# tjysdsg/speech-recognition

Hardware: AMD Instinct MI355X
Metric: frame-state loglik/s + utterances/s Viterbi decode (higher is better)
Workload: dtype f64; 1 GPU; configs[1]: 10-digit HMM, 5 states/digit, 8-mix GMM, 39-dim, 10000 utterances/GPU (999364 frames on rank 0), isolated-word decode; states=50, mixtures=8, dim=39, parallelism=utterance-sharded x1, batches_in_flight=2, process_group=single

## Files before the change

include/gmmhmm.h:

```cpp
#ifndef GMMHMM_H
#define GMMHMM_H

#include <stdint.h>

#ifdef __cplusplus
extern "C" {
#endif

typedef enum {
    GH_OK = 0,
    GH_ERR_INVALID = -1,
    GH_ERR_HIP = -2,
    GH_ERR_NOMEM = -3,
    GH_ERR_NODEVICE = -4,
    GH_ERR_SELF_POINTER = -5,
    GH_ERR_UNSUPPORTED = -6,
    GH_ERR_COMM = -7
} gh_status;

typedef enum { GH_F32 = 0, GH_F64 = 1 } gh_dtype;

typedef struct gh_ctx gh_ctx;
typedef struct gh_gmm gh_gmm;
typedef struct gh_batch gh_batch;
// ... 71 lines not shown
void* gh_loglik_dev_ptr(gh_batch* b);
int gh_loglik_fetch(gh_ctx* ctx, const gh_batch* b, void* out_host );
int gh_component_loglik(gh_ctx* ctx, const gh_gmm* g, int state, int64_t N,
                        const double* x_host , double* out_host );
int gh_distance_matrix(gh_ctx* ctx, int64_t N, int K, int D, const double* x_host ,
                       const double* y_host , const double* var_host, int var_rows,
                       double* out_host );

int gh_lattices_create(gh_ctx* ctx, int L,
                       const int64_t* row_off , const int32_t* row_state,
                       const int64_t* arc_off , const int32_t* arc_to,
                       const int32_t* arc_from, const double* arc_cost,
                       const int64_t* start_off , const int32_t* start_rows,
                       const int64_t* end_off , const int32_t* end_rows,
                       gh_lattices** out);
int gh_lattices_create_transcripts(gh_ctx* ctx, int W, int n, const double* word_trans ,
                                   const int32_t* state_base , int64_t L,
                                   const int64_t* label_off , const int32_t* labels, gh_lattices** out);
void gh_lattices_destroy(gh_lattices* l);
int gh_lattices_set_beam(gh_lattices* l, int beam);

int gh_lattices_forms(const gh_lattices* l);

int gh_viterbi(gh_ctx* ctx, const gh_lattices* lat, const gh_batch* b,
               const int32_t* utt_lattice ,
               double* out_end_cost, int32_t* out_best_end,
               int32_t* out_path, const int64_t* path_off , int32_t* out_path_len,
               double* out_costs, const int64_t* costs_off );
int gh_viterbi_fused(gh_ctx* ctx, const gh_gmm* g, const gh_lattices* lat, gh_batch* b, int log_domain,
                     double* out_end_cost, int32_t* out_best_end,
                     int32_t* out_path, const int64_t* path_off , int32_t* out_path_len,
                     double* out_costs, const int64_t* costs_off );
int gh_ctx_last_fused(const gh_ctx* ctx);
int64_t gh_viterbi_path_cap(const gh_lattices* lat, int l, int64_t T);
int gh_viterbi_labels(gh_ctx* ctx, const gh_lattices* lat, const gh_batch* b,
                      const int32_t* utt_lattice , const int32_t* row_label,
                      double* out_end_cost, int32_t* out_best_end,
                      int32_t* out_labels, const int64_t* label_off , int32_t* out_n_labels);
int gh_viterbi_labels_timed(gh_ctx* ctx, const gh_lattices* lat, const gh_batch* b,
                            const int32_t* utt_lattice , const int32_t* row_label,
                            double* out_end_cost, int32_t* out_best_end,
                            int32_t* out_labels, const int64_t* label_off , int32_t* out_n_labels,
                            int32_t* out_begin );

#define GH_SEGMENT_START (1 << 30)
int gh_align_segments(gh_ctx* ctx, const gh_lattices* lat, const gh_batch* b,
                      const int32_t* utt_lattice ,
                      double* out_end_cost, int32_t* out_best_end, int32_t* out_frame_state );
int gh_align_runs(gh_ctx* ctx, const gh_lattices* lat, const gh_batch* b, const int32_t* utt_lattice ,
                  double* out_end_cost, int32_t* out_best_end, int run_cap, int32_t* out_runs ,
                  int32_t* out_run_cnt );

int gh_viterbi_labels_packed(gh_ctx* ctx, const gh_lattices* lat, const gh_batch* b,
                             const int32_t* utt_lattice , const int32_t* row_label, int max_labels,
                             double* out_end_cost, int32_t* out_best_end,
                             int32_t* out_labels, int64_t out_capacity, int32_t* out_n_labels);
int gh_viterbi_labels_packed_timed(gh_ctx* ctx, const gh_lattices* lat, const gh_batch* b,
                                   const int32_t* utt_lattice , const int32_t* row_label, int max_labels,
                                   double* out_end_cost, int32_t* out_best_end,
                                   int32_t* out_labels, int64_t out_capacity, int32_t* out_n_labels,
                                   int32_t* out_begin );

int gh_dtw(gh_ctx* ctx, const gh_batch* b, int n, const double* y, const double* var,
           const double* trans, int beam, const double* dist_host,
           double* out_costs, int32_t* out_path, int32_t* out_path_len);

// ... 165 lines not shown
```

speech-recognition_amd/csrc/gh_decode.hip:

```cpp
#include "gh_internal.h"
#include <chrono>
#include <string>
#include "gh_host.h"
#include "gh_viterbi.h"
#include "gh_dtw.h"
#include "gh_fb.h"

namespace {

template <bool TIMED>
__device__ __forceinline__ void path_labels_walk(const int32_t* __restrict__ path, const int64_t* __restrict__ path_off,
                                                 const int32_t* __restrict__ path_len, const int32_t* __restrict__ utt_lat,
                                                 const gh_lattices::desc* __restrict__ descs,
                                                 const int32_t* __restrict__ row_label,
                                                 const int64_t* __restrict__ label_off, int32_t* __restrict__ labels,
                                                 int32_t* __restrict__ n_labels, int* __restrict__ flag,
                                                 int32_t* __restrict__ begins) {
    const int64_t u = blockIdx.x;
    const int lane = threadIdx.x;
    const int len = path_len[u];
    const int32_t* p = path + 2 * path_off[u];
    const int32_t* lab = row_label + descs[utt_lat ? utt_lat[u] : 0].row_base;
    const int64_t cap = label_off[u + 1] - label_off[u];
    int32_t* out = labels + label_off[u];
// ... 548 lines not shown
    }
    return GH_OK;
}

extern "C" int gh_viterbi(gh_ctx* ctx, const gh_lattices* lat, const gh_batch* b, const int32_t* utt_lattice,
                          double* out_end_cost, int32_t* out_best_end, int32_t* out_path,
                          const int64_t* path_off, int32_t* out_path_len, double* out_costs,
                          const int64_t* costs_off) {
    return viterbi_impl(ctx, lat, b, utt_lattice, out_end_cost, out_best_end, out_path, path_off, out_path_len, out_costs,
                        costs_off, nullptr, nullptr, nullptr, nullptr);
}

extern "C" int gh_viterbi_fused(gh_ctx* ctx, const gh_gmm* g, const gh_lattices* lat, gh_batch* b, int log_domain,
                                double* out_end_cost, int32_t* out_best_end, int32_t* out_path, const int64_t* path_off,
                                int32_t* out_path_len, double* out_costs, const int64_t* costs_off) {
    GH_REQUIRE(ctx && g && lat && b, "gh_viterbi_fused: NULL argument");
    GH_REQUIRE(g->D == b->D || b->N == 0, "gh_viterbi_fused: model has %d dimensions, batch %d", g->D, b->D);
    ctx->last_fused = 0;
    bool can = g->M == 1 && lat->chain_ok && lat->beam <= 0 && forced_kernel() == 0 && gh_fused_dv(g->D) > 0 && !lat->deferred_src;
    if (const char* e = getenv("GMMHMM_FUSED")) can = can && atoi(e) != 0;
    if (b->any_T1) can = false;
    if (!can) {
        const int compat = ctx->compat;
        if (log_domain) ctx->compat &= ~1;
        const int rc = gh_loglik(ctx, g, b, nullptr);
        ctx->compat = compat;
        if (rc) return rc;
    }
    return viterbi_impl(ctx, lat, b, nullptr, out_end_cost, out_best_end, out_path, path_off, out_path_len, out_costs, costs_off,
                        nullptr, nullptr, nullptr, nullptr, -1, nullptr, can ? g : nullptr, log_domain);
}

extern "C" int gh_ctx_last_fused(const gh_ctx* ctx) { return ctx ? ctx->last_fused : -1; }

extern "C" int gh_viterbi_labels_timed(gh_ctx* ctx, const gh_lattices* lat, const gh_batch* b, const int32_t* utt_lattice,
                                       const int32_t* row_label, double* out_end_cost, int32_t* out_best_end,
                                       int32_t* out_labels, const int64_t* label_off, int32_t* out_n_labels, int32_t* out_begin) {
    GH_REQUIRE(row_label && out_labels && label_off && out_n_labels, "gh_viterbi_labels: NULL argument");
    return viterbi_impl(ctx, lat, b, utt_lattice, out_end_cost, out_best_end, nullptr, nullptr, nullptr, nullptr, nullptr,
                        row_label, out_labels, label_off, out_n_labels, -1, nullptr, nullptr, 0, 0, nullptr, nullptr, out_begin);
}

extern "C" int gh_viterbi_labels(gh_ctx* ctx, const gh_lattices* lat, const gh_batch* b, const int32_t* utt_lattice,
                                 const int32_t* row_label, double* out_end_cost, int32_t* out_best_end,
                                 int32_t* out_labels, const int64_t* label_off, int32_t* out_n_labels) {
    return gh_viterbi_labels_timed(ctx, lat, b, utt_lattice, row_label, out_end_cost, out_best_end, out_labels, label_off, out_n_labels,
                                   nullptr);
}

extern "C" int gh_dtw(gh_ctx* ctx, const gh_batch* b, int n, const double* y, const double* var,
                      const double* trans, int beam, const double* dist_host, double* out_costs,
                      int32_t* out_path, int32_t* out_path_len) {
    GH_REQUIRE(ctx && b && trans, "gh_dtw: NULL argument");
    GH_REQUIRE(dist_host || y, "gh_dtw: need template rows or a distance matrix");
    GH_REQUIRE(n > 1 && n <= 1024, "gh_dtw: n=%d (2..1024 supported; decode.py:22 asserts n > 1)", n);
    GH_REQUIRE(b->dtype == GH_F64 || dist_host, "gh_dtw: built-in distances need an fp64 batch");
    GH_REQUIRE(!out_path || out_path_len, "gh_dtw: out_path needs out_path_len");
    GH_HIP(hipSetDevice(ctx->device));
    const int64_t U = b->U, N = b->N;
    const int D = b->D;
    if (U == 0) return GH_OK;
    for (int64_t u = 0; u < U; ++u)
        GH_REQUIRE(b->offsets[u + 1] - b->offsets[u] > 1, "gh_dtw: utterance %lld has fewer than 2 frames (decode.py:22)",
                   (long long)u);
    std::vector<double> logdet(n, 0.0);
    if (var && !dist_host)
// ... 344 lines not shown
```

speech-recognition_amd/csrc/gh_internal.h:

```cpp
#pragma once
#include <hip/hip_runtime.h>
#include <stdint.h>
#include <stdarg.h>
#include <stdio.h>
#include <string>
#include <vector>
#include "../../include/gmmhmm.h"

void gh_set_error(const char* fmt, ...);

#define GH_HIP(call)                                                                     \
    do {                                                                                 \
        hipError_t e_ = (call);                                                          \
        if (e_ != hipSuccess) {                                                          \
            gh_set_error("%s:%d %s -> %s", __FILE__, __LINE__, #call, hipGetErrorString(e_)); \
            return (e_ == hipErrorOutOfMemory) ? GH_ERR_NOMEM : GH_ERR_HIP;              \
        }                                                                                \
    } while (0)

#define GH_REQUIRE(cond, ...)                 \
    do {                                      \
        if (!(cond)) {                        \
            gh_set_error(__VA_ARGS__);        \
            return GH_ERR_INVALID;            \
        }                                     \
    } while (0)

#define GH_LEAN_NARROW_ARCS 3

#define GH_LSE_SCALE64 184.66496523378731614
#define GH_LSE_SCALE32 1.4426950408889634074
#define GH_LSE_OFF64 (-1e300)
#define GH_LSE_OFF32 (-1e30f)

struct gh_ctx {
    int device;
    hipStream_t stream;
    int n_cu;
    void* scratch;
    size_t scratch_bytes;
    int* d_flag;
    void* pinned;
    size_t pinned_bytes;
    double* d_fp64_tables;
    int compat;
    int last_fused = 0;
    int last_chunks;
    size_t budget_cache = 0;
    int budget_age = 0;
    void* fit_arena = nullptr;
    size_t fit_arena_bytes = 0;
    void* fit_pin = nullptr;
    void* fit_act = nullptr;
    size_t fit_act_bytes = 0;
};

int gh_scratch(gh_ctx* ctx, size_t bytes, void** out);
size_t gh_scratch_budget(gh_ctx* ctx, bool fresh = false);
int gh_pinned(gh_ctx* ctx, size_t bytes, void** out);

struct gh_gmm {
    gh_ctx* ctx;
    void* d_arena;
    int S, M, D, KP;
    std::vector<double> hA, hB, hC;
    bool host_stale = false;
    double *dA64, *dB64, *dC64;
    float *dA32, *dB32, *dC32;
    float* dCen32;
    double *dMean, *dIvar, *dLogc;
    int* dAnyPos = nullptr;
    int any_pos_host = -1;
    int M_pad, n_tiles;
    double *dApk64, *dCpk64;
    float *dApk32, *dCpk32;
    uint64_t serial = 0;
};
uint64_t gh_next_serial();

// ... 192 lines not shown
```

speech-recognition_amd/csrc/gh_loglik_mfma.hip:

```cpp
#include <type_traits>
#include "gh_internal.h"
#include "gh_wave.h"

namespace {

typedef double v4d __attribute__((ext_vector_type(4)));
typedef float v4f __attribute__((ext_vector_type(4)));

struct gh_loglik_blk { int64_t n0; int32_t nrows, t0, t1, pad; };

template <typename T> struct Acc;
template <> struct Acc<double> {
    typedef v4d type;
    static __device__ __forceinline__ v4d mfma(double a, double b, v4d c) {
        return __builtin_amdgcn_mfma_f64_16x16x4f64(a, b, c, 0, 0, 0);
    }
};
template <> struct Acc<float> {
    typedef v4f type;
    static __device__ __forceinline__ v4f mfma(float a, float b, v4f c) {
        return __builtin_amdgcn_mfma_f32_16x16x4f32(a, b, c, 0, 0, 0);
    }
};

// ... 216 lines not shown
    } else {
        const bool last = (t + 1) % tiles_per_state == 0;
        const int s = t / tiles_per_state;
#pragma unroll
        for (int c = 0; c < 2; ++c) {
            T mx, sm;
            tile_lse<T, V>(c ? acc1 : acc0, 4, mx, sm, tab, k);
            const T d = run_mx[c] - mx;
            const T e = exp2s((d > T(0)) ? -d : d, tab, k.e3);
            run_sm[c] = (d > T(0)) ? fma(sm, e, run_sm[c]) : fma(run_sm[c], e, sm);
            run_mx[c] = (d > T(0)) ? run_mx[c] : mx;
        }
        const bool odd = q & 1;
        const T v = nll_of<T>(odd ? run_mx[1] : run_mx[0], odd ? run_sm[1] : run_sm[0], tab, inf_below, k);
        *((last && q < 2) ? (odd ? orow1 : orow0) + s : dummy) = v;
#pragma unroll
        for (int c = 0; c < 2; ++c) {
            run_mx[c] = last ? Dom<T>::off : run_mx[c];
            run_sm[c] = last ? T(0) : run_sm[c];
        }
    }
}

#ifndef GH_MF_SGB
#define GH_MF_SGB 0
#endif
template <typename T, int KS, int MP, bool MULTI, bool FE = false>
__global__ __launch_bounds__(64, (sizeof(T) == 4 ? 3 : 1)) void loglik_mfma_kernel(const T* __restrict__ X, int64_t N, int D,
                                                         const T* __restrict__ Apk, const T* __restrict__ Cpk,
                                                         int n_tiles, int S, int M_pad, int chunk_tiles,
                                                         const double* __restrict__ tables, int tab_off,
                                                         T* __restrict__ out, int bpw,
                                                         const gh_loglik_blk* __restrict__ blk_tab, int64_t n_blk,
                                                         const T* __restrict__ cen, T inf_below) {
    typedef typename Acc<T>::type V;
#ifndef GH_MF_RING32
#define GH_MF_RING32 2
#endif
#ifndef GH_MF_RING64
#define GH_MF_RING64 1
#endif
    constexpr int R = KS / (sizeof(T) == 4 ? GH_MF_RING32 : GH_MF_RING64);
    extern __shared__ __attribute__((aligned(16))) unsigned char smem_raw[];
    T* lds = reinterpret_cast<T*>(smem_raw);
    const int lane = threadIdx.x;
    const int f = lane & 15, q = lane >> 4;
    const int64_t n_blocks = (N + 31) / 32;
    int64_t n0 = (int64_t)blockIdx.x * (MULTI ? bpw : 1) * 32;
#ifdef GH_MF_TIMING
    long long tk[5], tw[2];
    tk[0] = clock64(); tw[0] = wall_clock64();
#endif
    int nrows = 0;
    const bool subset = MULTI && blk_tab != nullptr;
    const int64_t kb0 = (int64_t)blockIdx.x * (MULTI ? bpw : 1);
    int t_lo = subset ? blk_tab[kb0].t0 : 0, t_hi = n_tiles, nxt_t0 = 0;
    double* tab = reinterpret_cast<double*>(smem_raw + tab_off);
    if (sizeof(T) == 8 && MP != 1) {
        double tr[6];
#pragma unroll
        for (int it = 0; it < 6; ++it) tr[it] = tables[lane + 64 * it];
#pragma unroll
        for (int it = 0; it < 6; ++it) tab[lane + 64 * it] = tr[it];
    }
    auto stage_frames = [&]() {
        const int nelem = nrows * D;
        const T* src = X + n0 * D;
        T xr[KS];
#pragma unroll
        for (int it = 0; it < KS; ++it) {
            const int i = lane + 64 * it;
            xr[it] = (i < nelem) ? src[i] : T(0);
        }
#pragma unroll
        for (int it = 0; it < KS; ++it) {
            const int i = lane + 64 * it;
            if (i < nelem) lds[i] = xr[it];
        }
        __syncthreads();
    };
    constexpr int KQ = KS / 2;
    T b[2][KS];
    T cen_r[KQ];
#pragma unroll
    for (int j = 0; j < KQ; ++j) cen_r[j] = (sizeof(T) == 4 && cen) ? cen[4 * j + q] : T(0);
    auto build_b = [&]() {
#pragma unroll
        for (int c = 0; c < 2; ++c) {
            const int row = 16 * c + f;
#pragma unroll
            for (int j = 0; j < KQ; ++j) {
                const int d = 4 * j + q;
                T v = (row < nrows && d < D) ? lds[row * D + d] : T(0);
                if (sizeof(T) == 4) v = (row < nrows && d < D) ? v - cen_r[j] : T(0);
                b[c][j] = v * v;
                b[c][KQ + j] = v;
            }
        }
        __syncthreads();
    };

    const int tiles_per_state = (MP <= 16) ? 1 : M_pad / 16;
    const int SC = (MP <= 16) ? chunk_tiles * (16 / (MP <= 16 ? MP : 16)) : chunk_tiles / tiles_per_state;
    const int RS = (S <= SC) ? S : SC;
    T* dummy = lds + 32 * RS + lane;
    T run_mx[2] = {Dom<T>::off, Dom<T>::off}, run_sm[2] = {T(0), T(0)};
    LseK lse_k;
    if (sizeof(T) == 8 && !MULTI && !FE && MP != 1) lse_k.pin();
    int chunk_s0 = 0;
    int subset_cnt = 0;

    T ring[R];
#pragma unroll
    for (int j = 0; j < R; ++j) ring[j] = Apk[((int64_t)t_lo * KS + j) * 64 + lane];
    V c_a, c_b, p0, p1;
#pragma unroll
    for (int r = 0; r < 4; ++r) c_a[r] = Cpk[t_lo * 16 + 4 * q + r];

    auto mfma_tile = [&](int t, V& acc0, V& acc1, const V& c_use, V& c_load) {
        const int tn = (!MULTI || t + 1 < t_hi) ? t + 1 : nxt_t0;
        const global_ptr<T> cp = uniform_ptr(Cpk + (unsigned)(tn * 16));
#pragma unroll
        for (int r = 0; r < 4; ++r) c_load[r] = cp[4 * q + r];
        constexpr int WIN = 4096 / (64 * (int)sizeof(T)), NW = (KS + WIN - 1) / WIN;
        global_ptr<T> a_cur[NW], a_nxt[NW];
#pragma unroll
        for (int w = 0; w < NW; ++w) {
            a_cur[w] = uniform_ptr(Apk + (unsigned)(t * (KS * 64) + w * (WIN * 64)));
            a_nxt[w] = uniform_ptr(Apk + (unsigned)(tn * (KS * 64) + w * (WIN * 64)));
        }
#pragma unroll
        for (int ks = 0; ks < KS; ++ks) {
            const T a = ring[ks % R];
#ifdef GH_MF_NOMFMA
            if (ks == 0) { acc0 = c_use; acc1 = c_use; }
            if (ks % 8 == 0) { acc0[ks % 4] += a * b[0][ks]; acc1[ks % 4] += a * b[1][ks]; }
            else asm volatile("" :: "v"(a));
#else
            acc0 = Acc<T>::mfma(a, b[0][ks], ks == 0 ? c_use : acc0);
            acc1 = Acc<T>::mfma(a, b[1][ks], ks == 0 ? c_use : acc1);
#endif
#ifndef GH_MF_NOLOAD
            ring[ks % R] = (ks + R < KS) ? a_cur[(ks + R) / WIN][((ks + R) % WIN) * 64 + lane]
                                         : a_nxt[(ks + R - KS) / WIN][((ks + R - KS) % WIN) * 64 + lane];
#endif
        }
    };
    auto flush = [&]() {
        const int cnt = subset ? subset_cnt : ((chunk_s0 + SC < S) ? chunk_s0 + SC : S) - chunk_s0;
        __syncthreads();
        if (cnt == S && !subset) {
            typedef T V16 __attribute__((ext_vector_type(16 / sizeof(T))));
            constexpr int VE = 16 / sizeof(T);
            T* dst = out + n0 * S;
            const int total = nrows * S;
            const int nvec = total / VE;
#pragma unroll 4
            for (int i = lane; i < nvec; i += 64)
                reinterpret_cast<V16*>(dst)[i] = reinterpret_cast<const V16*>(lds)[i];
            for (int i = nvec * VE + lane; i < total; i += 64) dst[i] = lds[i];
        } else if (cnt > 0) {
            const int total = nrows * cnt;
            for (int i = lane; i < total; i += 64) {
                const int r = i / cnt, j = i - r * cnt;
                out[(n0 + r) * S + chunk_s0 + j] = lds[r * RS + j];
            }
        }
        __syncthreads();
        chunk_s0 += SC;
    };

    const int nb = MULTI ? bpw : 1;
    int64_t staged_n0 = -1;
    for (int ib = 0; ib < nb; ++ib, n0 += 32) {
        if (subset) {
            const int64_t k = kb0 + ib;
            if (k >= n_blk) break;
            const gh_loglik_blk bd = blk_tab[k];
            n0 = bd.n0; nrows = bd.nrows; t_lo = bd.t0; t_hi = bd.t1;
            nxt_t0 = (ib + 1 < nb && k + 1 < n_blk) ? blk_tab[k + 1].t0 : bd.t0;
        } else {
            if (MULTI && n0 >= N) break;
            nrows = (int)((N - n0 < 32) ? (N - n0) : 32);
        }
        if (!(subset && ib > 0 && n0 == staged_n0)) {
#ifdef GH_MF_PRIO
            __builtin_amdgcn_s_setprio(3);
#endif
            stage_frames();
            build_b();
#ifdef GH_MF_PRIO
            __builtin_amdgcn_s_setprio(0);
#endif
            staged_n0 = n0;
        }
        chunk_s0 = (MP <= 16) ? t_lo * (16 / (MP <= 16 ? MP : 16)) : t_lo / tiles_per_state;
        if (subset) {
            const int s_end = (MP <= 16) ? t_hi * (16 / (MP <= 16 ? MP : 16)) : t_hi / tiles_per_state;
            subset_cnt = ((s_end < S) ? s_end : S) - chunk_s0;
        }
#ifdef GH_MF_TIMING
        tk[1] = clock64();
        tk[2] = tk[1];
#endif
        auto epi = [&](const V& e0, const V& e1, int t, auto chk) {
            tile_epilogue<T, V, MP, FE, decltype(chk)::value>(e0, e1, t, f, q, S, RS, chunk_s0, tiles_per_state, lds, dummy, tab, run_mx, run_sm, inf_below, lse_k);
#pragma unroll
            for (int i = 0; i < (GH_MF_SGB ? 2 * KS : 0); ++i) {
                __builtin_amdgcn_sched_group_barrier(0x008, 1, 0);
                __builtin_amdgcn_sched_group_barrier(0x002, sizeof(T) == 8 ? 5 : 3, 0);
            }
            if (!subset && (t + 1) % chunk_tiles == 0 && t + 1 < n_tiles) flush();
        };
        V r0, r1;
        const int tb = MULTI ? t_lo : 0, te = MULTI ? t_hi : n_tiles;
        mfma_tile(tb, p0, p1, c_a, c_b);
        if (sizeof(T) == 8) {
            int t = tb + 1;
            for (; t + 1 < te; t += 2) {
                mfma_tile(t, r0, r1, c_b, c_a);
                epi(p0, p1, t - 1, std::false_type());
                mfma_tile(t + 1, p0, p1, c_a, c_b);
                epi(r0, r1, t, std::false_type());
            }
            if (t < te) {
                mfma_tile(t, r0, r1, c_b, c_a);
                epi(p0, p1, t - 1, std::false_type());
                epi(r0, r1, t, std::true_type());
            } else {
                epi(p0, p1, te - 1, std::true_type());
                if (MULTI) c_a = c_b;
            }
        } else {
            for (int t = tb + 1; t < te; ++t) {
                mfma_tile(t, r0, r1, c_b, c_a);
                epi(p0, p1, t - 1, std::false_type());
                p0 = r0;
                p1 = r1;
                c_b = c_a;
            }
            epi(p0, p1, te - 1, std::true_type());
            if (MULTI) c_a = c_b;
        }
#ifdef GH_MF_TIMING
        tk[3] = clock64();
#endif
        flush();
#ifdef GH_MF_TIMING
// ... 35 lines not shown
        for (int64_t r = r0; r < r1; ++r) {
            const int lo = st_lo[r], hi = st_hi[r];
            if (lo < 0 || hi > S || lo >= hi) { gh_set_error("gh_loglik_subset: utterance %lld has state range [%d, %d)", (long long)u, lo, hi); return GH_ERR_INVALID; }
            int t0, t1;
            if (M_pad <= 16) { const int spt = 16 / M_pad; t0 = lo / spt; t1 = (hi + spt - 1) / spt; }
            else { const int tps = M_pad / 16; t0 = lo * tps; t1 = hi * tps; }
            runs.push_back({t0, t1});
        }
        std::sort(runs.begin(), runs.end());
        size_t w = 0;
        for (size_t i = 0; i < runs.size(); ++i) {
            if (w > 0 && runs[i].first <= runs[w - 1].second) runs[w - 1].second = std::max(runs[w - 1].second, runs[i].second);
            else runs[w++] = runs[i];
        }
        runs.resize(w);
        for (const auto& tr : runs) {
            const int t0 = tr.first, t1 = tr.second;
            const int span = (M_pad <= 16) ? (t1 - t0) * (16 / M_pad) : (t1 - t0) / (M_pad / 16);
            if (span > SC) return 1;
            max_tiles = std::max(max_tiles, t1 - t0);
        }
        for (int64_t f = b->offsets[u]; f < b->offsets[u + 1]; f += 32)
            for (const auto& tr : runs)
                tabv.push_back(gh_loglik_blk{f, (int32_t)std::min<int64_t>(32, b->offsets[u + 1] - f), tr.first, tr.second, 0});
    }
    *max_tiles_out = max_tiles;
    return GH_OK;
}

template <typename T>
int launch_mfma_t(gh_ctx* ctx, const gh_gmm* g, gh_batch* b, const T* Apk, const T* Cpk, const int32_t* st_lo,
                  const int32_t* st_hi, const T* cen, const int64_t* rng_off, const gh_loglik_plan* plan) {
    const int64_t N = b->N;
    if (N == 0) return GH_OK;
    const int KS = g->KP / 2;
    const int M_pad = g->M_pad, n_tiles = g->n_tiles, S = g->S;
    int chunk_tiles, SC;
    chunk_shape(g, &chunk_tiles, &SC);
    size_t lds = ((size_t)32 * std::max(std::min(SC, S), g->D) + 64) * sizeof(T);
    lds = (lds + 15) & ~size_t(15);
    const int tab_off = (int)lds;
    if (sizeof(T) == 8 && M_pad != 1) lds += 384 * sizeof(double);
    const double* tables = ctx->d_fp64_tables;
    const T inf_below = (ctx->compat & 1) ? (T)(-745.1332191019412 * (sizeof(T) == 8 ? GH_LSE_SCALE64 : GH_LSE_SCALE32)) : Dom<T>::off_test;
    gh_loglik_blk* d_blk = nullptr;
    int64_t n_blk = 0;
    int max_tiles = n_tiles;
    if (plan) {
        d_blk = static_cast<gh_loglik_blk*>(plan->d_blk);
        n_blk = plan->n_blk;
        max_tiles = plan->max_tiles;
        if (n_blk == 0) return GH_OK;
    } else if (st_lo) {
        std::vector<gh_loglik_blk> tabv;
        int rc = build_blk_table(g, b, SC, st_lo, st_hi, rng_off, tabv, &max_tiles);
        if (rc) return rc;
        n_blk = (int64_t)tabv.size();
        if (n_blk == 0) return GH_OK;
        void* base;
        rc = gh_scratch(ctx, tabv.size() * sizeof(gh_loglik_blk), &base);
        if (rc) return rc;
        d_blk = static_cast<gh_loglik_blk*>(base);
        GH_HIP(hipMemcpyAsync(d_blk, tabv.data(), tabv.size() * sizeof(gh_loglik_blk), hipMemcpyHostToDevice, ctx->stream));
        GH_HIP(hipStreamSynchronize(ctx->stream));
    }
    const bool subset = plan || st_lo;
    const int64_t n_blocks = subset ? n_blk : (N + 31) / 32;
    const int per_block = std::max(1, max_tiles * KS * 2);
    int bpw = (int)std::max<int64_t>(1, std::min<int64_t>(8, (512 + per_block - 1) / per_block));
    if (const char* e = getenv("GMMHMM_LOGLIK_BPW")) bpw = std::max(1, std::min(16, atoi(e)));
    if (subset) bpw = std::max(bpw, 2);
    const unsigned grid = (unsigned)((n_blocks + bpw - 1) / bpw);
    const T* X = static_cast<const T*>(b->feats);
    T* out = static_cast<T*>(b->nll);
    const bool fe = sizeof(T) == 8 && (ctx->compat & 2) && M_pad >= 4;
#define GH_MF_LAUNCH(ks, mp)                                                                                             \
    do {                                                                                                                 \
        if (fe && sizeof(T) == 8 && mp >= 4) {                                                                           \
            if (bpw > 1)                                                                                                 \
                hipLaunchKernelGGL((loglik_mfma_kernel<T, ks, mp, true, (sizeof(T) == 8 && mp >= 4)>), dim3(grid), dim3(64), lds, ctx->stream, X, N, g->D, \
                                   Apk, Cpk, n_tiles, S, M_pad, chunk_tiles, tables, tab_off, out, bpw, d_blk, n_blk, cen, inf_below); \
            else                                                                                                         \
                hipLaunchKernelGGL((loglik_mfma_kernel<T, ks, mp, false, (sizeof(T) == 8 && mp >= 4)>), dim3(grid), dim3(64), lds, ctx->stream, X, N, g->D, \
                                   Apk, Cpk, n_tiles, S, M_pad, chunk_tiles, tables, tab_off, out, bpw, d_blk, n_blk, cen, inf_below); \
        } else if (bpw > 1)                                                                                                     \
            hipLaunchKernelGGL((loglik_mfma_kernel<T, ks, mp, true>), dim3(grid), dim3(64), lds, ctx->stream, X, N, g->D, \
                               Apk, Cpk, n_tiles, S, M_pad, chunk_tiles, tables, tab_off, out, bpw, d_blk, n_blk, cen, inf_below); \
        else                                                                                                             \
            hipLaunchKernelGGL((loglik_mfma_kernel<T, ks, mp, false>), dim3(grid), dim3(64), lds, ctx->stream, X, N, g->D, \
                               Apk, Cpk, n_tiles, S, M_pad, chunk_tiles, tables, tab_off, out, bpw, d_blk, n_blk, cen, inf_below); \
    } while (0)
#define GH_MF_CASE(ks)                                   \
    case ks:                                             \
        switch (M_pad) {                                 \
            case 1: GH_MF_LAUNCH(ks, 1); break;          \
            case 2: GH_MF_LAUNCH(ks, 2); break;          \
            case 4: GH_MF_LAUNCH(ks, 4); break;          \
            case 8: GH_MF_LAUNCH(ks, 8); break;          \
            case 16: GH_MF_LAUNCH(ks, 16); break;        \
            default: GH_MF_LAUNCH(ks, 32); break;        \
        }                                                \
        break;
    switch (KS) {
        GH_MF_CASE(2)
        GH_MF_CASE(4)
        GH_MF_CASE(8)
        GH_MF_CASE(12)
        GH_MF_CASE(20)
        GH_MF_CASE(24)
        GH_MF_CASE(32)
        default:
            return 1;
    }
#undef GH_MF_CASE
#undef GH_MF_LAUNCH
    GH_HIP(hipGetLastError());
    return GH_OK;
}

}

int gh_launch_loglik_mfma(gh_ctx* ctx, const gh_gmm* g, gh_batch* b, const int32_t* st_lo, const int32_t* st_hi,
                          const int64_t* rng_off, const gh_loglik_plan* plan) {
// ... 29 lines not shown
```

speech-recognition_amd/sr/recognition/_hip.py:

```python
import ctypes as C
import os
import threading

import numpy as np

_HERE = os.path.dirname(os.path.abspath(__file__))
LIB_PATH = os.environ.get("GMMHMM_LIB") or os.path.normpath(
    os.path.join(_HERE, "..", "..", "lib", "libgmmhmm.so"))

GH_F32, GH_F64 = 0, 1
GH_ERR_SELF_POINTER = -5
GH_ERR_UNSUPPORTED = -6
GH_ERR_COMM = -7

_c_i32p = C.POINTER(C.c_int32)
_c_i64p = C.POINTER(C.c_int64)
_c_f64p = C.POINTER(C.c_double)
_c_u8p = C.POINTER(C.c_uint8)


class EndpointParams(C.Structure):
    _fields_ = [("width", C.c_int32), ("stride", C.c_int32), ("speech_frames", C.c_int32), ("silence_frames", C.c_int32),
                ("forget", C.c_double), ("adjustment", C.c_double), ("onset", C.c_double), ("offset", C.c_double)]

# ... 36 lines not shown
    "gh_mfcc_frames": (C.c_int64, [C.c_int64, C.c_int, C.c_double]),
    "gh_mfcc": (C.c_int, [C.c_void_p, C.c_int, C.c_int, C.c_double, C.c_double, C.c_double, C.c_double, C.c_int64,
                          C.c_void_p, _c_i64p, _c_i64p, _c_f64p, _c_f64p]),
    "gh_batch_create_from_pcm": (C.c_int, [C.c_void_p, C.c_int, C.c_int, C.c_int, C.c_int, C.c_double, C.c_double,
                                           C.c_double, C.c_double, C.c_int64, C.c_void_p, _c_i64p, _c_i64p,
                                           C.POINTER(C.c_void_p)]),
    "gh_endpoint_frames": (C.c_int64, [C.c_int64, C.c_int, C.c_int]),
    "gh_endpoints": (C.c_int, [C.c_void_p, C.c_int64, C.c_void_p, _c_i64p, C.POINTER(EndpointParams), C.c_int, _c_i64p, _c_i64p,
                               _c_i32p, _c_u8p, _c_i64p, _c_i64p, _c_u8p, _c_f64p, _c_f64p, _c_f64p]),
    "gh_batch_create_from_pcm_endpointed": (C.c_int, [C.c_void_p, C.c_int, C.c_int, C.c_int, C.c_int, C.c_double, C.c_double,
                                                      C.c_double, C.c_double, C.c_int64, C.c_void_p, _c_i64p,
                                                      C.POINTER(EndpointParams), C.c_int, C.c_int, _c_i64p, _c_i64p, _c_i32p,
                                                      _c_u8p, _c_i64p, _c_i64p, C.POINTER(C.c_void_p)]),
    "gh_loglik": (C.c_int, [C.c_void_p, C.c_void_p, C.c_void_p, C.c_void_p]),
    "gh_loglik_sets": (C.c_int, [C.c_void_p, C.c_void_p, C.c_void_p, _c_i64p, _c_i32p, _c_i32p]),
    "gh_loglik_subset": (C.c_int, [C.c_void_p, C.c_void_p, C.c_void_p, _c_i32p, _c_i32p]),
    "gh_loglik_dev_ptr": (C.c_void_p, [C.c_void_p]),
    "gh_loglik_fetch": (C.c_int, [C.c_void_p, C.c_void_p, C.c_void_p]),
    "gh_component_loglik": (C.c_int, [C.c_void_p, C.c_void_p, C.c_int, C.c_int64, _c_f64p, _c_f64p]),
    "gh_distance_matrix": (C.c_int, [C.c_void_p, C.c_int64, C.c_int, C.c_int, _c_f64p, _c_f64p, _c_f64p,
                                     C.c_int, _c_f64p]),
    "gh_lattices_create": (C.c_int, [C.c_void_p, C.c_int, _c_i64p, _c_i32p, _c_i64p, _c_i32p, _c_i32p,
                                     _c_f64p, _c_i64p, _c_i32p, _c_i64p, _c_i32p, C.POINTER(C.c_void_p)]),
    "gh_lattices_create_transcripts": (C.c_int, [C.c_void_p, C.c_int, C.c_int, _c_f64p, _c_i32p, C.c_int64, _c_i64p, _c_i32p,
                                                 C.POINTER(C.c_void_p)]),
    "gh_lattices_destroy": (None, [C.c_void_p]),
    "gh_lattices_set_beam": (C.c_int, [C.c_void_p, C.c_int]),
    "gh_lattices_forms": (C.c_int, [C.c_void_p]),
    "gh_viterbi": (C.c_int, [C.c_void_p, C.c_void_p, C.c_void_p, _c_i32p, _c_f64p, _c_i32p, _c_i32p, _c_i64p,
                             _c_i32p, _c_f64p, _c_i64p]),
    "gh_viterbi_fused": (C.c_int, [C.c_void_p, C.c_void_p, C.c_void_p, C.c_void_p, C.c_int, _c_f64p, _c_i32p, _c_i32p, _c_i64p,
                                   _c_i32p, _c_f64p, _c_i64p]),
    "gh_ctx_last_fused": (C.c_int, [C.c_void_p]),
    "gh_viterbi_path_cap": (C.c_int64, [C.c_void_p, C.c_int, C.c_int64]),
    "gh_viterbi_labels": (C.c_int, [C.c_void_p, C.c_void_p, C.c_void_p, _c_i32p, _c_i32p, _c_f64p, _c_i32p, _c_i32p,
                                    _c_i64p, _c_i32p]),
    "gh_viterbi_labels_timed": (C.c_int, [C.c_void_p, C.c_void_p, C.c_void_p, _c_i32p, _c_i32p, _c_f64p, _c_i32p, _c_i32p,
                                    _c_i64p, _c_i32p, _c_i32p]),
    "gh_align_segments": (C.c_int, [C.c_void_p, C.c_void_p, C.c_void_p, _c_i32p, _c_f64p, _c_i32p, _c_i32p]),
    "gh_align_runs": (C.c_int, [C.c_void_p, C.c_void_p, C.c_void_p, _c_i32p, _c_f64p, _c_i32p, C.c_int, _c_i32p, _c_i32p]),
    "gh_viterbi_labels_packed": (C.c_int, [C.c_void_p, C.c_void_p, C.c_void_p, _c_i32p, _c_i32p, C.c_int, _c_f64p, _c_i32p,
                                           _c_i32p, C.c_int64, _c_i32p]),
    "gh_viterbi_labels_packed_timed": (C.c_int, [C.c_void_p, C.c_void_p, C.c_void_p, _c_i32p, _c_i32p, C.c_int, _c_f64p, _c_i32p,
                                           _c_i32p, C.c_int64, _c_i32p, _c_i32p]),
    "gh_dtw": (C.c_int, [C.c_void_p, C.c_void_p, C.c_int, _c_f64p, _c_f64p, _c_f64p, C.c_int, _c_f64p,
                         _c_f64p, _c_i32p, _c_i32p]),
    "gh_kmeans_assign": (C.c_int, [C.c_void_p, C.c_void_p, C.c_int64, C.c_int64, C.c_int, _c_f64p, _c_f64p,
                                   _c_i32p]),
    "gh_kmeans_resident_clusters": (C.c_int, [C.c_void_p, C.c_void_p, C.c_int, _c_i32p]),
    "gh_kmeans_assign_multi": (C.c_int, [C.c_void_p, C.c_void_p, C.c_int, _c_i64p, C.POINTER(C.c_uint8), C.c_int, _c_f64p,
                                         _c_f64p, _c_i32p, _c_i32p, _c_f64p]),
    "gh_em_accumulate_multi": (C.c_int, [C.c_void_p, C.c_void_p, C.c_int, _c_i64p, C.POINTER(C.c_uint8), C.c_int, _c_f64p,
                                         _c_f64p, _c_f64p, _c_f64p, _c_f64p, C.c_void_p]),
    "gh_forward_backward": (C.c_int, [C.c_void_p, C.c_void_p, C.c_void_p, _c_i32p, C.c_int, _c_f64p, _c_f64p, _c_f64p,
                                      _c_f64p, _c_i64p, _c_f64p, _c_f64p]),
    "gh_bw_accumulate": (C.c_int, [C.c_void_p, C.c_void_p, C.c_void_p, C.c_double, _c_f64p, C.c_void_p]),
    "gh_em_accumulate": (C.c_int, [C.c_void_p, C.c_void_p, C.c_int64, C.c_int64, C.c_int, _c_f64p, _c_f64p,
                                   _c_f64p, _c_f64p, _c_f64p]),
    "gh_gmm_update": (C.c_int, [C.c_void_p, C.c_void_p, _c_f64p, _c_f64p, _c_f64p]),
    "gh_em_create": (C.c_int, [C.c_void_p, C.c_void_p, C.c_int, C.c_int, C.c_int, _c_f64p, _c_f64p, _c_f64p, _c_f64p, _c_i32p,
                               C.c_double, C.c_double, C.c_double, C.c_int, C.POINTER(C.c_void_p)]),
    "gh_em_create_transcripts": (C.c_int, [C.c_void_p, C.c_void_p, C.c_int, C.c_int, C.c_int, _c_f64p, _c_f64p, _c_f64p, _c_f64p,
                                           C.c_int64, _c_i64p, _c_i32p, _c_i32p, C.c_double, C.c_double, C.c_double, C.c_int,
                                           C.POINTER(C.c_void_p)]),
    "gh_em_destroy": (None, [C.c_void_p]),
    "gh_em_iteration": (C.c_int, [C.c_void_p, C.c_void_p, C.c_void_p, _c_f64p]),
# ... 130 lines not shown
        if rc == GH_ERR_COMM:
            raise CommError("libgmmhmm error %d: %s" % (rc, msg))
        raise BackendError("libgmmhmm error %d: %s" % (rc, msg))


def _f64(a):
    return np.ascontiguousarray(a, dtype=np.float64)


def _ptr(a, typ):
    return None if a is None else a.ctypes.data_as(typ)


class Context:

    def __init__(self, device=0):
        self.lib = load_library()
        h = C.c_void_p()
        _check(self.lib, self.lib.gh_ctx_create(int(device), C.byref(h)))
        self.h = h
        self.device = int(device)

    def sync(self):
        _check(self.lib, self.lib.gh_ctx_sync(self.h))

    def set_compat(self, underflow=True, lse_f32=False):
        _check(self.lib, self.lib.gh_ctx_set_compat(self.h, (1 if underflow else 0) | (2 if lse_f32 else 0)))

    @property
    def last_fused(self):
        return int(self.lib.gh_ctx_last_fused(self.h)) == 1

    @property
    def last_chunks(self):
        return int(self.lib.gh_ctx_last_chunks(self.h))

    def device_sync(self):
        _check(self.lib, self.lib.gh_device_sync(self.h))

    @property
    def stream(self):
        return self.lib.gh_ctx_stream(self.h)

    def new_event(self):
        e = C.c_void_p()
        _check(self.lib, self.lib.gh_event_create(self.h, C.byref(e)))
        return e

    def record(self, event):
        _check(self.lib, self.lib.gh_event_record(self.h, event))

    def wait_event(self, event):
        _check(self.lib, self.lib.gh_ctx_wait_event(self.h, event))

    def elapsed_ms(self, start, stop):
        ms = C.c_float()
        _check(self.lib, self.lib.gh_event_elapsed_ms(start, stop, C.byref(ms)))
        return float(ms.value)

    def close(self):
        if getattr(self, "h", None):
            self.lib.gh_ctx_destroy(self.h)
            self.h = None

    def __del__(self):
        try:
# ... 1476 lines not shown
```

Before: 43.49 billion frame-state loglik/s.

## Split tail loglik workgroups across state ranges and add unguarded full-tile staging

Adds an optional tail mode, enabled through GMMHMM_LOGLIK_TAIL, where the last frame blocks of the MFMA loglik grid are each split across several workgroups covering disjoint state-tile ranges. The aim is to fill the device during the final wave. It also adds a fast path for full 32-row frame blocks that drops the per-element bounds checks when staging frames into LDS and building the B operands. The tail split is off by default, so only the full-tile fast path and the minor tb/te change are active by default. A counter exposing the tail size is added for inspection.

```diff
diff --git a/include/gmmhmm.h b/include/gmmhmm.h
--- a/include/gmmhmm.h
+++ b/include/gmmhmm.h
@@ -127,6 +127,7 @@
                      int32_t* out_path, const int64_t* path_off , int32_t* out_path_len,
                      double* out_costs, const int64_t* costs_off );
 int gh_ctx_last_fused(const gh_ctx* ctx);
+int gh_ctx_last_loglik_tail(const gh_ctx* ctx);
 int64_t gh_viterbi_path_cap(const gh_lattices* lat, int l, int64_t T);
 int gh_viterbi_labels(gh_ctx* ctx, const gh_lattices* lat, const gh_batch* b,
                       const int32_t* utt_lattice , const int32_t* row_label,
diff --git a/speech-recognition_amd/csrc/gh_decode.hip b/speech-recognition_amd/csrc/gh_decode.hip
--- a/speech-recognition_amd/csrc/gh_decode.hip
+++ b/speech-recognition_amd/csrc/gh_decode.hip
@@ -604,6 +604,7 @@
 }
 
 extern "C" int gh_ctx_last_fused(const gh_ctx* ctx) { return ctx ? ctx->last_fused : -1; }
+extern "C" int gh_ctx_last_loglik_tail(const gh_ctx* ctx) { return ctx ? ctx->last_loglik_tail : -1; }
 
 extern "C" int gh_viterbi_labels_timed(gh_ctx* ctx, const gh_lattices* lat, const gh_batch* b, const int32_t* utt_lattice,
                                        const int32_t* row_label, double* out_end_cost, int32_t* out_best_end,
diff --git a/speech-recognition_amd/csrc/gh_internal.h b/speech-recognition_amd/csrc/gh_internal.h
--- a/speech-recognition_amd/csrc/gh_internal.h
+++ b/speech-recognition_amd/csrc/gh_internal.h
@@ -45,6 +45,7 @@
     double* d_fp64_tables;
     int compat;
     int last_fused = 0;
+    int last_loglik_tail = 0;
     int last_chunks;
     size_t budget_cache = 0;
     int budget_age = 0;
diff --git a/speech-recognition_amd/csrc/gh_loglik_mfma.hip b/speech-recognition_amd/csrc/gh_loglik_mfma.hip
--- a/speech-recognition_amd/csrc/gh_loglik_mfma.hip
+++ b/speech-recognition_amd/csrc/gh_loglik_mfma.hip
@@ -272,7 +272,8 @@
                                                          const double* __restrict__ tables, int tab_off,
                                                          T* __restrict__ out, int bpw,
                                                          const gh_loglik_blk* __restrict__ blk_tab, int64_t n_blk,
-                                                         const T* __restrict__ cen, T inf_below) {
+                                                         const T* __restrict__ cen, T inf_below,
+                                                         unsigned tail_wg0, int tail_parts) {
     typedef typename Acc<T>::type V;
 #ifndef GH_MF_RING32
 #define GH_MF_RING32 2
@@ -285,8 +286,14 @@
     T* lds = reinterpret_cast<T*>(smem_raw);
     const int lane = threadIdx.x;
     const int f = lane & 15, q = lane >> 4;
-    const int64_t n_blocks = (N + 31) / 32;
+    const bool tail = !MULTI && blockIdx.x >= tail_wg0;
+    unsigned tail_part = 0;
     int64_t n0 = (int64_t)blockIdx.x * (MULTI ? bpw : 1) * 32;
+    if (tail) {
+        const unsigned k = blockIdx.x - tail_wg0, kb = k / (unsigned)tail_parts;
+        tail_part = k - kb * (unsigned)tail_parts;
+        n0 = ((int64_t)tail_wg0 + kb) * 32;
+    }
 #ifdef GH_MF_TIMING
     long long tk[5], tw[2];
     tk[0] = clock64(); tw[0] = wall_clock64();
@@ -295,6 +302,12 @@
     const bool subset = MULTI && blk_tab != nullptr;
     const int64_t kb0 = (int64_t)blockIdx.x * (MULTI ? bpw : 1);
     int t_lo = subset ? blk_tab[kb0].t0 : 0, t_hi = n_tiles, nxt_t0 = 0;
+    const int tiles_per_state = (MP <= 16) ? 1 : M_pad / 16;
+    if (tail) {
+        const unsigned units = (unsigned)(n_tiles / tiles_per_state);
+        t_lo = (int)(tail_part * units / (unsigned)tail_parts) * tiles_per_state;
+        t_hi = (int)((tail_part + 1) * units / (unsigned)tail_parts) * tiles_per_state;
+    }
     double* tab = reinterpret_cast<double*>(smem_raw + tab_off);
     if (sizeof(T) == 8 && MP != 1) {
         double tr[6];
@@ -303,19 +316,31 @@
 #pragma unroll
         for (int it = 0; it < 6; ++it) tab[lane + 64 * it] = tr[it];
     }
+    bool full = false;
     auto stage_frames = [&]() {
         const int nelem = nrows * D;
         const T* src = X + n0 * D;
         T xr[KS];
-#pragma unroll
-        for (int it = 0; it < KS; ++it) {
-            const int i = lane + 64 * it;
-            xr[it] = (i < nelem) ? src[i] : T(0);
-        }
-#pragma unroll
-        for (int it = 0; it < KS; ++it) {
-            const int i = lane + 64 * it;
-            if (i < nelem) lds[i] = xr[it];
+#ifndef GH_MF_NOFULL
+        full = nrows == 32 && D >= 2 * KS - 2;
+#endif
+        if (full) {
+#pragma unroll
+            for (int it = 0; it < KS - 1; ++it) xr[it] = src[lane + 64 * it];
+            xr[KS - 1] = (lane + 64 * (KS - 1) < nelem) ? src[lane + 64 * (KS - 1)] : T(0);
+#pragma unroll
+            for (int it = 0; it < KS; ++it) lds[lane + 64 * it] = xr[it];
+        } else {
+#pragma unroll
+            for (int it = 0; it < KS; ++it) {
+                const int i = lane + 64 * it;
+                xr[it] = (i < nelem) ? src[i] : T(0);
+            }
+#pragma unroll
+            for (int it = 0; it < KS; ++it) {
+                const int i = lane + 64 * it;
+                if (i < nelem) lds[i] = xr[it];
+            }
         }
         __syncthreads();
     };
@@ -325,22 +350,37 @@
 #pragma unroll
     for (int j = 0; j < KQ; ++j) cen_r[j] = (sizeof(T) == 4 && cen) ? cen[4 * j + q] : T(0);
     auto build_b = [&]() {
-#pragma unroll
-        for (int c = 0; c < 2; ++c) {
-            const int row = 16 * c + f;
-#pragma unroll
-            for (int j = 0; j < KQ; ++j) {
-                const int d = 4 * j + q;
-                T v = (row < nrows && d < D) ? lds[row * D + d] : T(0);
-                if (sizeof(T) == 4) v = (row < nrows && d < D) ? v - cen_r[j] : T(0);
-                b[c][j] = v * v;
-                b[c][KQ + j] = v;
+        if (full) {
+#pragma unroll
+            for (int c = 0; c < 2; ++c) {
+                const int row = 16 * c + f;
+#pragma unroll
+                for (int j = 0; j < KQ; ++j) {
+                    const int d = 4 * j + q;
+                    const bool in = j + 1 < KQ || d < D;
+                    T v = in ? lds[row * D + d] : T(0);
+                    if (sizeof(T) == 4) v = in ? v - cen_r[j] : T(0);
+                    b[c][j] = v * v;
+                    b[c][KQ + j] = v;
+                }
+            }
+        } else {
+#pragma unroll
+            for (int c = 0; c < 2; ++c) {
+                const int row = 16 * c + f;
+#pragma unroll
+                for (int j = 0; j < KQ; ++j) {
+                    const int d = 4 * j + q;
+                    T v = (row < nrows && d < D) ? lds[row * D + d] : T(0);
+                    if (sizeof(T) == 4) v = (row < nrows && d < D) ? v - cen_r[j] : T(0);
+                    b[c][j] = v * v;
+                    b[c][KQ + j] = v;
+                }
             }
         }
         __syncthreads();
     };
 
-    const int tiles_per_state = (MP <= 16) ? 1 : M_pad / 16;
     const int SC = (MP <= 16) ? chunk_tiles * (16 / (MP <= 16 ? MP : 16)) : chunk_tiles / tiles_per_state;
     const int RS = (S <= SC) ? S : SC;
     T* dummy = lds + 32 * RS + lane;
@@ -387,9 +427,10 @@
         }
     };
     auto flush = [&]() {
-        const int cnt = subset ? subset_cnt : ((chunk_s0 + SC < S) ? chunk_s0 + SC : S) - chunk_s0;
+        const bool ranged = subset || tail;
+        const int cnt = ranged ? subset_cnt : ((chunk_s0 + SC < S) ? chunk_s0 + SC : S) - chunk_s0;
         __syncthreads();
-        if (cnt == S && !subset) {
+        if (cnt == S && !ranged) {
             typedef T V16 __attribute__((ext_vector_type(16 / sizeof(T))));
             constexpr int VE = 16 / sizeof(T);
             T* dst = out + n0 * S;
@@ -435,7 +476,7 @@
             staged_n0 = n0;
         }
         chunk_s0 = (MP <= 16) ? t_lo * (16 / (MP <= 16 ? MP : 16)) : t_lo / tiles_per_state;
-        if (subset) {
+        if (subset || tail) {
             const int s_end = (MP <= 16) ? t_hi * (16 / (MP <= 16 ? MP : 16)) : t_hi / tiles_per_state;
             subset_cnt = ((s_end < S) ? s_end : S) - chunk_s0;
         }
@@ -453,7 +494,9 @@
             if (!subset && (t + 1) % chunk_tiles == 0 && t + 1 < n_tiles) flush();
         };
         V r0, r1;
-        const int tb = MULTI ? t_lo : 0, te = MULTI ? t_hi : n_tiles;
+        const int tb = t_lo, te = t_hi;
+        __builtin_assume(tb >= 0);
+        __builtin_assume(te <= n_tiles);
         mfma_tile(tb, p0, p1, c_a, c_b);
         if (sizeof(T) == 8) {
             int t = tb + 1;
@@ -555,6 +598,7 @@
 int launch_mfma_t(gh_ctx* ctx, const gh_gmm* g, gh_batch* b, const T* Apk, const T* Cpk, const int32_t* st_lo,
                   const int32_t* st_hi, const T* cen, const int64_t* rng_off, const gh_loglik_plan* plan) {
     const int64_t N = b->N;
+    ctx->last_loglik_tail = 0;
     if (N == 0) return GH_OK;
     const int KS = g->KP / 2;
     const int M_pad = g->M_pad, n_tiles = g->n_tiles, S = g->S;
@@ -593,7 +637,24 @@
     int bpw = (int)std::max<int64_t>(1, std::min<int64_t>(8, (512 + per_block - 1) / per_block));
     if (const char* e = getenv("GMMHMM_LOGLIK_BPW")) bpw = std::max(1, std::min(16, atoi(e)));
     if (subset) bpw = std::max(bpw, 2);
-    const unsigned grid = (unsigned)((n_blocks + bpw - 1) / bpw);
+    const int tail_units = n_tiles / (M_pad <= 16 ? 1 : M_pad / 16);
+    int64_t n_tail = 0;
+    int parts = 1;
+    if (const char* e = getenv("GMMHMM_LOGLIK_TAIL")) {
+        long long nt = 0;
+        int np = 1;
+        const int got = sscanf(e, "%lld,%d", &nt, &np);
+        n_tail = (got >= 1 && nt > 0) ? nt : 0;
+        parts = (got >= 2) ? np : 2;
+    }
+    parts = std::min(parts, tail_units);
+    if (subset || bpw != 1 || S > SC || parts < 2) n_tail = 0;
+    n_tail = std::min(n_tail, n_blocks);
+    if (n_blocks + n_tail * (parts - 1) > 0x7fffffff) n_tail = 0;
+    if (n_tail == 0) parts = 1;
+    const unsigned grid = (unsigned)((n_blocks + bpw - 1) / bpw + n_tail * (parts - 1));
+    const unsigned tail_wg0 = (unsigned)((n_blocks + bpw - 1) / bpw - n_tail);
+    ctx->last_loglik_tail = (int)std::min<int64_t>(n_tail * parts, 0x7fffffff);
     const T* X = static_cast<const T*>(b->feats);
     T* out = static_cast<T*>(b->nll);
     const bool fe = sizeof(T) == 8 && (ctx->compat & 2) && M_pad >= 4;
@@ -602,16 +663,16 @@
         if (fe && sizeof(T) == 8 && mp >= 4) {                                                                           \
             if (bpw > 1)                                                                                                 \
                 hipLaunchKernelGGL((loglik_mfma_kernel<T, ks, mp, true, (sizeof(T) == 8 && mp >= 4)>), dim3(grid), dim3(64), lds, ctx->stream, X, N, g->D, \
-                                   Apk, Cpk, n_tiles, S, M_pad, chunk_tiles, tables, tab_off, out, bpw, d_blk, n_blk, cen, inf_below); \
+                                   Apk, Cpk, n_tiles, S, M_pad, chunk_tiles, tables, tab_off, out, bpw, d_blk, n_blk, cen, inf_below, tail_wg0, parts); \
             else                                                                                                         \
                 hipLaunchKernelGGL((loglik_mfma_kernel<T, ks, mp, false, (sizeof(T) == 8 && mp >= 4)>), dim3(grid), dim3(64), lds, ctx->stream, X, N, g->D, \
-                                   Apk, Cpk, n_tiles, S, M_pad, chunk_tiles, tables, tab_off, out, bpw, d_blk, n_blk, cen, inf_below); \
+                                   Apk, Cpk, n_tiles, S, M_pad, chunk_tiles, tables, tab_off, out, bpw, d_blk, n_blk, cen, inf_below, tail_wg0, parts); \
         } else if (bpw > 1)                                                                                                     \
             hipLaunchKernelGGL((loglik_mfma_kernel<T, ks, mp, true>), dim3(grid), dim3(64), lds, ctx->stream, X, N, g->D, \
-                               Apk, Cpk, n_tiles, S, M_pad, chunk_tiles, tables, tab_off, out, bpw, d_blk, n_blk, cen, inf_below); \
+                               Apk, Cpk, n_tiles, S, M_pad, chunk_tiles, tables, tab_off, out, bpw, d_blk, n_blk, cen, inf_below, tail_wg0, parts); \
         else                                                                                                             \
             hipLaunchKernelGGL((loglik_mfma_kernel<T, ks, mp, false>), dim3(grid), dim3(64), lds, ctx->stream, X, N, g->D, \
-                               Apk, Cpk, n_tiles, S, M_pad, chunk_tiles, tables, tab_off, out, bpw, d_blk, n_blk, cen, inf_below); \
+                               Apk, Cpk, n_tiles, S, M_pad, chunk_tiles, tables, tab_off, out, bpw, d_blk, n_blk, cen, inf_below, tail_wg0, parts); \
     } while (0)
 #define GH_MF_CASE(ks)                                   \
     case ks:                                             \
diff --git a/speech-recognition_amd/sr/recognition/_hip.py b/speech-recognition_amd/sr/recognition/_hip.py
--- a/speech-recognition_amd/sr/recognition/_hip.py
+++ b/speech-recognition_amd/sr/recognition/_hip.py
@@ -92,6 +92,7 @@
     "gh_viterbi_fused": (C.c_int, [C.c_void_p, C.c_void_p, C.c_void_p, C.c_void_p, C.c_int, _c_f64p, _c_i32p, _c_i32p, _c_i64p,
                                    _c_i32p, _c_f64p, _c_i64p]),
     "gh_ctx_last_fused": (C.c_int, [C.c_void_p]),
+    "gh_ctx_last_loglik_tail": (C.c_int, [C.c_void_p]),
     "gh_viterbi_path_cap": (C.c_int64, [C.c_void_p, C.c_int, C.c_int64]),
     "gh_viterbi_labels": (C.c_int, [C.c_void_p, C.c_void_p, C.c_void_p, _c_i32p, _c_i32p, _c_f64p, _c_i32p, _c_i32p,
                                     _c_i64p, _c_i32p]),
@@ -288,6 +289,10 @@
         return int(self.lib.gh_ctx_last_fused(self.h)) == 1
 
     @property
+    def last_loglik_tail(self):
+        return int(self.lib.gh_ctx_last_loglik_tail(self.h))
+
+    @property
     def last_chunks(self):
         return int(self.lib.gh_ctx_last_chunks(self.h))
 
```

Result: no change. 43.53 billion frame-state loglik/s (median of 2 runs) (+0.1%).
